# samedii/perceptor

Measured on AMD Instinct MI355X. Metric: denoising steps/sec (UNet+CLIP-grad) at 512x512 batch 8, higher is better.
Workload: dtype bf16

## Files before the change

### perceptor_amd/csrc/build.py

```python
from __future__ import annotations

import os
import subprocess
import sys
from concurrent.futures import ThreadPoolExecutor

HERE = os.path.dirname(os.path.abspath(__file__))
LIB = os.path.join(HERE, "libperceptor_hip.so")
SOURCES = ["igemm.hip", "conv3x3.hip", "conv_wd.hip", "gemm_wd.hip", "norm.hip", "attn.hip", "attn_flash.hip", "elementwise.hip", "clip.hip", "f32gemm.hip", "sampling.hip", "backward.hip", "resnet.hip"]
FLAGS = ["-O3", "--offload-arch=gfx950", "-std=c++17", "-fPIC"]
FILE_FLAGS = {"conv_wd.hip": ["-fno-slp-vectorize"]}


def _stale(out: str, deps) -> bool:
    if not os.path.exists(out):
        return True
    t = os.path.getmtime(out)
    return any(os.path.getmtime(d) > t for d in deps)


def build(force: bool = False, verbose: bool = False, variant: str = "", extra_flags=()) -> str:
    hipcc = os.environ.get("HIPCC", "/opt/rocm/bin/hipcc")
    lib = LIB if not variant else LIB.replace(".so", f"_{variant}.so")
    bdir = "build" if not variant else f"build_{variant}"
    hdrs = [os.path.join(HERE, "common.h"), os.path.join(HERE, "..", "..", "include", "perceptor_hip.h")]
    srcs = [s for s in SOURCES if os.path.exists(os.path.join(HERE, s))]
    objs = []

    def compile_one(src):
        obj = os.path.join(HERE, bdir, src.replace(".hip", ".o"))
        os.makedirs(os.path.dirname(obj), exist_ok=True)
        if force or _stale(obj, [os.path.join(HERE, src)] + hdrs):
            cmd = [hipcc, *FLAGS, *FILE_FLAGS.get(src, []), *extra_flags, "-c", os.path.join(HERE, src), "-o", obj]
            if verbose:
                print(" ".join(cmd), flush=True)
            subprocess.run(cmd, check=True)
        return obj

    with ThreadPoolExecutor(max_workers=min(7, len(srcs))) as ex:
        objs = list(ex.map(compile_one, srcs))
    if force or _stale(lib, objs):
        cmd = [hipcc, "--offload-arch=gfx950", "-shared", "-fPIC", "-o", lib, *objs]
        if verbose:
            print(" ".join(cmd), flush=True)
# ... 10 lines not shown
```

### perceptor_amd/csrc/conv3x3.hip

```cpp
#include "common.h"
#include "epilogue.h"
#include "../../include/perceptor_hip.h"

namespace {

constexpr int PW = 34;

__device__ __forceinline__ int swz(int row, int chunk) { return row * 128 + ((chunk ^ ((row >> 1) & 7)) << 4); }

template <typename T, int WM, int WN, int PRO, bool EARLY, int NJ = 4, int NWB = 2>
__global__ __launch_bounds__(WM * WN * 64, 2) void conv3x3_halo_kernel(const pmi_igemm_args a) {
  constexpr int XB = 2;
  constexpr int TH = WM * XB;
  constexpr int NT = WM * WN * 64;
  constexpr int RPI = NT / 8;
  constexpr int BN = WN * NJ * 32;
  constexpr int PP = (TH + 2) * PW;
  constexpr int NPI = (PP + RPI - 1) / RPI;
  constexpr int NWI = BN / RPI;
  constexpr int PATCH_BYTES = NPI * RPI * 128;
  constexpr int WBYTES = BN * 128;
  __shared__ __attribute__((aligned(16))) char smem[PATCH_BYTES + NWB * WBYTES];
  char* const wbuf = smem + PATCH_BYTES;

// ... 322 lines not shown
    const int tiles = nimg * (a.H / 8) * (a.W / 32) * ((a.N + 31) / 32);
    hipLaunchKernelGGL((conv3x3_halo_kernel<T, 4, 1, PRO, false, 1>), dim3(tiles), dim3(256), 0, s, a);
  } else {
    const int tiles = nimg * (a.H / 8) * (a.W / 32) * ((a.N + 127) / 128);
    hipLaunchKernelGGL((conv3x3_halo_kernel<T, 4, 1, PRO, false>), dim3(tiles), dim3(256), 0, s, a);
  }
  PMI_CHECK_LAUNCH();
  return PMI_OK;
}

template <typename T>
int launch_t(const pmi_igemm_args& a, hipStream_t s, int cfg) {
  if (!a.pro_a) return launch_p<T, 0>(a, s, cfg);
  switch (a.pro_act) {
    case PMI_ACT_NONE: return launch_p<T, 1 + PMI_ACT_NONE>(a, s, cfg);
    case PMI_ACT_RELU: return launch_p<T, 1 + PMI_ACT_RELU>(a, s, cfg);
    case PMI_ACT_SILU: return launch_p<T, 1 + PMI_ACT_SILU>(a, s, cfg);
    default: return PMI_ERR_ARG;
  }
}

}

static int g_prefer0 = 1;
static int g_force_cfg = -1;
static int g_wd = 1;
static int g_wd128 = 1;
static int g_wd_mf16 = 1;
void pmi_conv3x3_allow_wd(int v) { g_wd = v; }
void pmi_conv3x3_wd_mf16(int v) { g_wd_mf16 = v; }
void pmi_conv3x3_wd128(int v) { g_wd128 = v; }
static int g_wd_smallc = 1;
void pmi_conv3x3_wd_smallc(int v) { g_wd_smallc = v; }
void pmi_conv3x3_force_config(int cfg) { g_force_cfg = cfg; }
void pmi_conv3x3_prefer_256(int v) { g_prefer0 = v; }

extern "C" int pmi_conv3x3_halo_config(const pmi_igemm_args* a) {
  if (a->taps != 9 || a->stride != 1 || a->batch > 1) return -1;
  const int Cin = a->C0 + a->C1;
  if (a->Bf && g_wd && g_wd_mf16 && g_wd_smallc && a->C1 == 0 && !a->A1 && a->C0 <= 32 && (a->C0 % 8) == 0 && !a->up && (a->W % 32) == 0 && (a->H % 8) == 0 && !a->pro_a &&
      ((!a->split_out && !a->split_in) || (a->split_out == 32 && a->split_in == 1 && (a->N % 128) == 0 && a->dtype != PMI_DT_BF16)) &&
      !a->out_f32 && !(a->R && a->res_f32) && (a->N % 32) == 0 && a->N >= 64 && (g_force_cfg < 0 || g_force_cfg == 8) &&
      (long)(a->M / (a->H * a->W)) * (a->H / 8) * (a->W / 32) * ((a->N + 127) / 128) >= (g_force_cfg == 8 ? 1 : 256))
    return 8;
  if ((Cin % 64) || (a->C0 % 64) || (a->W % 32) || (a->H % 8)) return -1;
  const bool plain_k = a->split_in == 1 && !a->split_out && !a->pro_a && a->out_f32 && a->N <= 32;
  if ((a->split_out || a->split_in) && !plain_k) {
    if (!a->Bf || !g_wd || !g_wd_mf16 || a->split_out != 32 || a->out_f32 || (a->N % 128) || a->dtype == PMI_DT_BF16) return -1;
    if (a->split_in == 2 && !a->pro_a) return -1;
    if (a->pro_a && (a->pro_act != PMI_ACT_SILU || !a->split_in)) return -1;
    const int cin_l = a->split_in == 1 ? Cin / 2 : Cin;
    const int t8s = a->M / (a->H * a->W) * (a->H / 8) * (a->W / 32);
    const bool ok6 = (a->N % 256) == 0 && (!a->pro_a || cin_l <= 2048), ok7 = !a->pro_a || cin_l <= 1024;
    if (g_force_cfg == 6 || g_force_cfg == 7) return (g_force_cfg == 6 ? ok6 : ok7) ? g_force_cfg : -1;
    if (g_force_cfg >= 0) return -1;
    if (ok6 && t8s * (a->N / 256) >= 192) return 6;
    if (g_wd128 && ok7 && t8s * (a->N / 128) >= 128) return 7;
    return -1;
  }
  if (a->N <= 32 && (a->N % 4) == 0 && !a->stats && !a->res_up && a->M / (a->H * a->W) * (a->H / 8) * (a->W / 32) >= 256) return 3;
  if (a->out_f32 || (a->R && a->res_f32)) return -1;
  if (a->N % 128) {
    const int t8 = a->M / (a->H * a->W) * (a->H / 8) * (a->W / 32);
    const bool ok7t = a->Bf && g_wd && g_wd_mf16 && (a->N % 32) == 0 && (a->N % 128) >= 64 && a->N > 128 && (!a->pro_a || a->C0 + a->C1 <= 1024);
    if (g_force_cfg == 7) return ok7t ? 7 : -1;
    return (g_force_cfg < 0 && g_wd128 && ok7t && t8 * ((a->N + 127) / 128) >= 256) ? 7 : -1;
  }
  if (a->Bf && g_wd && (!a->pro_a || a->C0 + a->C1 <= 2048)) {
    const int t8 = a->M / (a->H * a->W) * (a->H / 8) * (a->W / 32);
    const bool ok4 = (a->N % 256) == 0;
    if (g_force_cfg == 4 && ok4) return 4;
    if (g_force_cfg == 6 && ok4) return 6;
    if (g_force_cfg < 0 && ok4 && t8 * (a->N / 256) >= 192) return g_wd_mf16 ? 6 : 4;
    const bool ok7 = g_wd_mf16 && (!a->pro_a || a->C0 + a->C1 <= 1024);
    if (g_force_cfg == 7 && ok7) return 7;
    if (g_force_cfg < 0 && g_wd128 && ok7 && !ok4 && t8 * (a->N / 128) >= (a->N > 512 ? 128 : 256)) return 7;
    if (g_force_cfg < 0 && g_wd128 && ok7 && ok4 && t8 * (a->N / 128) >= 128) return 7;
  }
  const bool ok0 = (a->N % 256) == 0 || a->N >= 256, ok1 = (a->H % 16) == 0;
  if (g_force_cfg == 0 && ok0) return 0;
  if (g_force_cfg == 1 && ok1) return 1;
  if (g_force_cfg == 2) return 2;
  const int nimg = a->M / (a->H * a->W);
  const int px_tiles8 = nimg * (a->H / 8) * (a->W / 32);
  if (g_prefer0 && (a->N % 256) == 0 && px_tiles8 * (a->N / 256) >= 256) return 0;
  if (px_tiles8 * (a->N / 128) >= 128) return 2;
  if ((a->N % 256) == 0) return px_tiles8 * (a->N / 256) >= 192 ? 0 : -1;
  if (ok1 && (px_tiles8 / 2) * (a->N / 128) >= 192) return 1;
  return -1;
}

int pmi_conv3x3_halo_launch(const pmi_igemm_args* a, int cfg, void* stream) {
  hipStream_t s = (hipStream_t)stream;
  return a->dtype == PMI_DT_BF16 ? launch_t<BF16>(*a, s, cfg) : launch_t<F16>(*a, s, cfg);
}
```

### perceptor_amd/csrc/igemm.hip

```cpp
#include <cstdio>
#include <cstdlib>
#include "common.h"
#include "epilogue.h"
#include "../../include/perceptor_hip.h"

namespace {

constexpr int BM = 128, BN = 128, BK = 64;
constexpr int TILE_BYTES = 128 * 128;
constexpr int STAGE_BYTES = 2 * TILE_BYTES;

__device__ __forceinline__ int lds_off(int row, int chunk) { return row * 128 + ((chunk ^ ((row >> 1) & 7)) << 4); }

template <typename T, bool CONV, bool KFAST, bool PHASED = false>
__global__ __launch_bounds__(256, 2) void igemm_kernel(const pmi_igemm_args a) {
  static_assert(!PHASED || CONV, "the phased geometry is a convolution");
  __shared__ __attribute__((aligned(16))) char smem[2 * STAGE_BYTES];

  const int tid = threadIdx.x, lane = tid & 63, wid = tid >> 6;
  const int wr = wid >> 1, wc = wid & 1;
#ifdef PMI_STAMPS
#define GSTAMP(k) do { if (tid == 0 && a.reserved == 77 && a.splitk <= 1) ((long long*)a.ws)[(int64_t)blockIdx.x * 8 + (k)] = (long long)wall_clock64(); } while (0)
#else
#define GSTAMP(k) do {} while (0)
// ... 477 lines not shown
template <typename T>
int launch(const pmi_igemm_args& a, hipStream_t s) {
  const bool phased = a.up == 2;
  const int tiles = (((phased ? a.M / 4 : a.M) + BM - 1) / BM) * ((a.N + BN - 1) / BN);
  const dim3 grid(tiles, phased ? 4 : 1, a.batch > 1 ? a.batch : (a.splitk > 1 ? a.splitk : 1)), block(256);
  const bool conv = a.taps != 1 || a.up || a.stride == 2;
  const int Cin = a.C0 + a.C1;
  const bool kfast = (Cin % BK == 0) && (a.C0 % BK == 0);
  if (phased) {
    if (kfast) hipLaunchKernelGGL((igemm_kernel<T, true, true, true>), grid, block, 0, s, a);
    else hipLaunchKernelGGL((igemm_kernel<T, true, false, true>), grid, block, 0, s, a);
  } else if (conv) {
    if (kfast) hipLaunchKernelGGL((igemm_kernel<T, true, true>), grid, block, 0, s, a);
    else hipLaunchKernelGGL((igemm_kernel<T, true, false>), grid, block, 0, s, a);
  } else {
    if (kfast) hipLaunchKernelGGL((igemm_kernel<T, false, true>), grid, block, 0, s, a);
    else hipLaunchKernelGGL((igemm_kernel<T, false, false>), grid, block, 0, s, a);
  }
  PMI_CHECK_LAUNCH();
  if (a.splitk > 1) {
    const int64_t work = (int64_t)a.M * (a.N / 4);
    const int blocks = (int)((work + 255) / 256 > 4096 ? 4096 : (work + 255) / 256);
    hipLaunchKernelGGL(splitk_reduce_kernel<T>, dim3(blocks), dim3(256), 0, s, a);
    PMI_CHECK_LAUNCH();
  }
  return PMI_OK;
}

}

extern "C" int pmi_conv3x3_halo_config(const pmi_igemm_args* a);
int pmi_conv3x3_halo_launch(const pmi_igemm_args* a, int cfg, void* stream);
int pmi_conv3x3_wd_launch(const pmi_igemm_args* a, int cfg, void* stream);
extern "C" int pmi_gemm_wd_eligible(const pmi_igemm_args* a);
int pmi_gemm_wd_tile_rows(const pmi_igemm_args* a, int splitk);
int pmi_gemm_wd_launch(const pmi_igemm_args* a, void* stream);
void pmi_conv3x3_allow_wd(int v);
void pmi_conv3x3_wd_mf16(int v);
void pmi_conv3x3_wd128(int v);
void pmi_conv3x3_force_config(int cfg);
void pmi_conv3x3_prefer_256(int v);
static int g_allow_halo = 1;
static int g_wd_max_split = 8;
int pmi_conv3x3_wd_splitk(const pmi_igemm_args* a, int cfg);
extern "C" int pmi_igemm_splitk(const pmi_igemm_args* a) {
  if (a->batch > 1 || (a->N & 3) || a->up == 2) return 1;
  if (g_allow_halo) {
    const int halo = pmi_conv3x3_halo_config(a);
    if (halo >= 0) return pmi_conv3x3_wd_splitk(a, halo);
  }
  if (a->act == PMI_ACT_GEGLU) return 1;
  if (a->A1 && a->taps == 1 && pmi_gemm_wd_eligible(a)) return 1;
  if (pmi_gemm_wd_eligible(a)) {
    const int nch = (a->K + 127) / 128;
    int best = 1;
    long best_cost = -1;
    for (int s = 1; s <= g_wd_max_split && nch / s >= 4; s *= 2) {
      const int rows = pmi_gemm_wd_tile_rows(a, s);
      const long wgs = (long)((a->M + rows - 1) / rows) * (a->N < 256 ? 1 : (a->N + 255) / 256) * s;
      const long cost = ((wgs + 255) / 256) * rows * (nch / s + 6) + (s > 1 ? 8L * 144 : 0);
      if (best_cost < 0 || cost < best_cost) { best_cost = cost; best = s; }
    }
    return best;
  }
  const int tiles = ((a->M + BM - 1) / BM) * ((a->N + BN - 1) / BN);
  const int nk = (a->K + BK - 1) / BK;
  if (tiles >= 384 || nk < 16) return 1;
  int s = 512 / tiles;
  if (s > nk / 8) s = nk / 8;
  if (s > 16) s = 16;
  return s < 2 ? 1 : s;
}

int pmi_igemm_halo_allowed(void) { return g_allow_halo; }

extern "C" int pmi_igemm_stats_rows(const pmi_igemm_args* a) {
  if (a->batch > 1 || a->splitk > 1 || a->up == 2) return 0;
  const int halo = g_allow_halo ? pmi_conv3x3_halo_config(a) : -1;
  if (a->split_out) return halo >= 6 ? (a->H / 8) * (a->W / 32) : 0;
  if (halo == 3) return 0;
  if (halo >= 0) return (a->H / (halo == 1 ? 16 : 8)) * (a->W / 32);
  if (a->hw > 0 && (a->hw % BM) == 0 && (a->M % a->hw) == 0) return a->hw / BM;
  return 0;
}

void pmi_attn_flash_qt(int v);
void pmi_attn_flash_kv_chunks(int v);
void pmi_conv3x3_wd_splitk_enable(int v);
void pmi_gemm_wd_few_wgs(int v);
void pmi_conv3x3_wd_smallc(int v);

extern "C" int pmi_set_option(int key, int value) {
  if (key == 0) { const int old = g_allow_halo; g_allow_halo = value; return old; }
  if (key == 1) { pmi_conv3x3_force_config(value); return 0; }
  if (key == 2) { pmi_conv3x3_prefer_256(value); return 0; }
  if (key == 6) { pmi_conv3x3_allow_wd(value); return 0; }
  if (key == 7) { pmi_conv3x3_wd_mf16(value); return 0; }
  if (key == 8) { pmi_conv3x3_wd128(value); return 0; }
  if (key == 9) { pmi_attn_flash_qt(value); return 0; }
  if (key == 10) { pmi_conv3x3_wd_splitk_enable(value); return 0; }
  if (key == 11) { g_wd_max_split = value; return 0; }
  if (key == 12) { pmi_gemm_wd_few_wgs(value); return 0; }
  if (key == 13) { pmi_conv3x3_wd_smallc(value); return 0; }
  if (key == 14) { pmi_attn_flash_kv_chunks(value); return 0; }
  return PMI_ERR_ARG;
}

static int bad_arg(int line) {
  if (getenv("PMI_DEBUG")) fprintf(stderr, "pmi_igemm: argument check at igemm.hip:%d failed\n", line);
  return PMI_ERR_ARG;
}

extern "C" int pmi_igemm(const pmi_igemm_args* a, pmi_stream_t stream) {
  if (!a || !a->A0 || !a->B || !a->D) return bad_arg(__LINE__);
  if (a->M <= 0 || a->N <= 0 || a->K <= 0) return bad_arg(__LINE__);
  if ((a->K & 7) || (a->C0 & 7) || (a->C1 & 7)) return bad_arg(__LINE__);
  if ((a->N & 3) && (a->bias || a->nbias || a->R || a->ldd < ((a->N + 3) & ~3))) return bad_arg(__LINE__);
  if ((a->lda0 & 7) || (a->ldb & 7) || (a->ldd & 3)) return bad_arg(__LINE__);
  if (a->C1 > 0 && (!a->A1 || (a->lda1 & 7))) return bad_arg(__LINE__);
  if (a->taps != 1 && a->taps != 9 && a->taps != 16) return bad_arg(__LINE__);
  if (a->taps == 16 && (a->stride != 2 || a->up || a->res_up || a->Hin != 2 * a->H || a->Win != 2 * a->W)) return bad_arg(__LINE__);
  if (a->stride != 1 && a->stride != 2) return bad_arg(__LINE__);
  if (a->up == 2 && (a->taps != 9 || a->stride != 2 || a->res_up || a->A1 || a->C1 || a->R || a->nbias || a->stats || a->splitk > 1 || a->batch > 1 ||
                     a->split_out || a->split_in || a->pro_a || a->D2 || a->aux || a->dtype == PMI_DT_F16X2 || (a->M & 3))) return bad_arg(__LINE__);
  if (a->K != a->taps * (a->C0 + a->C1)) return bad_arg(__LINE__);
  if (a->R && (a->ldr & 3)) return bad_arg(__LINE__);
  if (a->split_out && ((a->split_out & 7) || a->split_out > 32 || a->out_f32 || (a->N % a->split_out) || a->batch > 1)) return bad_arg(__LINE__);
  if ((unsigned)a->split_in > 2u) return bad_arg(__LINE__);
  if (a->split_in == 2 && !a->split_out) return bad_arg(__LINE__);
  if (a->nbias && a->hw <= 0) return bad_arg(__LINE__);
  const bool conv = a->taps != 1 || a->up || a->stride == 2;
  if (a->res_up && ((a->H & 1) || (a->W & 1))) return bad_arg(__LINE__);
  if ((conv || a->res_up) && (a->H <= 0 || a->W <= 0 || a->Hin <= 0 || a->Win <= 0 || a->M % (a->H * a->W))) return bad_arg(__LINE__);
  if (a->up && (a->H != 2 * a->Hin || a->W != 2 * a->Win)) return bad_arg(__LINE__);
  if (a->batch > 1 && a->batch_inner <= 0) return bad_arg(__LINE__);
  const int halo = g_allow_halo ? pmi_conv3x3_halo_config(a) : -1;
  if (a->pro_a && (!a->pro_b || halo < 0)) return PMI_ERR_ARG;
  if ((a->split_in == 2 || ((a->split_in || a->split_out) && a->pro_a) || (a->split_out && a->R && a->res_f32)) && halo < 6) return bad_arg(__LINE__);
  if (a->stats && a->stats_p != pmi_igemm_stats_rows(a)) return PMI_ERR_ARG;
  if (a->splitk > 1 && (!a->ws || a->batch > 1 || (halo >= 0 && a->splitk != pmi_conv3x3_wd_splitk(a, halo)) || (a->N & 3) || a->stats)) return PMI_ERR_ARG;
  if (a->act == PMI_ACT_GEGLU && !pmi_gemm_wd_eligible(a)) return bad_arg(__LINE__);
  if ((a->D2 || a->aux) && !pmi_gemm_wd_eligible(a)) return bad_arg(__LINE__);
  if (pmi_gemm_wd_eligible(a) && !((a->nbias || a->res_up) && a->splitk <= 1)) {
    const int rc = pmi_gemm_wd_launch(a, stream);
    if (rc != PMI_OK || a->splitk <= 1 || a->reserved3 == 1) return rc;
    hipStream_t s = (hipStream_t)stream;
    const int64_t work = (int64_t)a->M * (a->N / 4);
    const int blocks = (int)((work + 255) / 256 > 4096 ? 4096 : (work + 255) / 256);
    if (a->dtype == PMI_DT_BF16) hipLaunchKernelGGL(splitk_reduce_kernel<BF16>, dim3(blocks), dim3(256), 0, s, *a);
    else hipLaunchKernelGGL(splitk_reduce_kernel<F16>, dim3(blocks), dim3(256), 0, s, *a);
    PMI_CHECK_LAUNCH();
    return PMI_OK;
  }
  if (halo >= 4) {
    const int rc = pmi_conv3x3_wd_launch(a, halo, stream);
    if (rc != PMI_OK || a->splitk <= 1) return rc;
    hipStream_t s = (hipStream_t)stream;
    const int64_t work = (int64_t)a->M * (a->N / 4);
    const int blocks = (int)((work + 255) / 256 > 4096 ? 4096 : (work + 255) / 256);
    if (a->dtype == PMI_DT_BF16) hipLaunchKernelGGL(splitk_reduce_kernel<BF16>, dim3(blocks), dim3(256), 0, s, *a);
    else hipLaunchKernelGGL(splitk_reduce_kernel<F16>, dim3(blocks), dim3(256), 0, s, *a);
    PMI_CHECK_LAUNCH();
    return PMI_OK;
  }
  if (halo >= 0) return pmi_conv3x3_halo_launch(a, halo, stream);
  hipStream_t s = (hipStream_t)stream;
  return a->dtype == PMI_DT_BF16 ? launch<BF16>(*a, s) : launch<F16>(*a, s);
}

extern "C" int pmi_abi_version(void) { return 1; }
```

### perceptor_amd/engine/adm.py

```python
from __future__ import annotations

from dataclasses import dataclass
from typing import Dict, List, Optional, Tuple

import torch

from .. import _hip
from .._hip import ACT_NONE, ACT_SILU, call, ptr
from . import ops
from .ops import PackedLinear


@dataclass(frozen=True)
class AdmConfig:
    image_size: int
    model_channels: int
    num_res_blocks: int
    channel_mult: Tuple[float, ...]
    attention_ds: Tuple[int, ...]
    num_heads: int = 1
    num_head_channels: int = -1
    num_heads_upsample: int = -1
    use_scale_shift_norm: bool = False
    resblock_updown: bool = False
# ... 113 lines not shown
                S[p + ".qkv.weight"] = (3 * l.c, l.c, 1); S[p + ".qkv.bias"] = (3 * l.c,)
                S[p + ".proj_out.weight"] = (l.c, l.c, 1); S[p + ".proj_out.bias"] = (l.c,)
            elif isinstance(l, _Resample) and cfg.conv_resample:
                n = l.p + (".conv" if l.up else ".op")
                S[n + ".weight"] = (l.c, l.c, 3, 3); S[n + ".bias"] = (l.c,)
    S["out.0.weight"] = (ch_last,); S["out.0.bias"] = (ch_last,)
    S["out.2.weight"] = (cfg.out_channels, int(cfg.channel_mult[0] * mc), 3, 3); S["out.2.bias"] = (cfg.out_channels,)
    return S


class AdmEngine:
    def __init__(self, cfg: AdmConfig, state_dict: Dict[str, torch.Tensor], device, dtype="bf16"):
        self.cfg, self.device = cfg, torch.device(device)
        self.dt = _hip.dtype_code(dtype)
        _hip.lib()
        sd, dev, dt = state_dict, self.device, self.dt
        self.inp, self.mid, self.out, self.ch_last = build_plan(cfg)
        f32 = lambda k: sd[k].detach().float().to(dev).contiguous()
        lin = lambda k, **kw: PackedLinear(sd[k + ".weight"], sd.get(k + ".bias"), dt, dev, **kw)
        self.w: Dict[str, object] = {}
        self.precise = dt == _hip.DT_F16X2
        if self.precise:
            self.te0, self.te2 = (f32("time_embed.0.weight"), f32("time_embed.0.bias")), (f32("time_embed.2.weight"), f32("time_embed.2.bias"))
        else:
            self.te0, self.te2 = lin("time_embed.0"), lin("time_embed.2")
        emb_w, emb_b, off = [], [], 0
        for layers in self.inp + [self.mid] + self.out:
            for l in layers:
                if isinstance(l, tuple):
                    self.w[l[1]] = lin(l[1], cin_pad=8)
                elif isinstance(l, _Res):
                    p = l.p
                    self.w[p + ".gn1"] = (f32(p + ".in_layers.0.weight"), f32(p + ".in_layers.0.bias"))
                    self.w[p + ".conv1"] = lin(p + ".in_layers.2", sources=l.srcs)
                    self.w[p + ".gn2"] = (f32(p + ".out_layers.0.weight"), f32(p + ".out_layers.0.bias"))
                    self.w[p + ".conv2"] = lin(p + ".out_layers.3")
                    if l.cin != l.cout:
                        self.w[p + ".skip"] = lin(p + ".skip_connection", sources=l.srcs)
                    l.emb_off = off
                    emb_w.append(sd[p + ".emb_layers.1.weight"].float()); emb_b.append(sd[p + ".emb_layers.1.bias"].float())
                    off += emb_w[-1].shape[0]
                elif isinstance(l, _Attn):
                    p = l.p
                    self.w[p + ".gn"] = (f32(p + ".norm.weight"), f32(p + ".norm.bias"))
                    self.w[p + ".qkv"] = lin(p + ".qkv")
                    self.w[p + ".proj"] = lin(p + ".proj_out")
                elif isinstance(l, _Resample) and cfg.conv_resample:
                    self.w[l.p] = lin(l.p + (".conv" if l.up else ".op"))
        if self.precise:
            self.emb_all = (torch.cat(emb_w, 0).to(dev).contiguous(), torch.cat(emb_b, 0).to(dev).contiguous())
        else:
            self.emb_all = PackedLinear(torch.cat(emb_w, 0), torch.cat(emb_b, 0), dt, dev)
        self.gn_out = (f32("out.0.weight"), f32("out.0.bias"))
        self.conv_out = lin("out.2")

    def _res(self, l: _Res, x, x1, emb):
        cfg, dt, w = self.cfg, self.dt, self.w
        g1, b1 = w[l.p + ".gn1"]
        ecols = 2 * l.cout if cfg.use_scale_shift_norm else l.cout
        e = emb[:, l.emb_off:l.emb_off + ecols]
        nb = None if cfg.use_scale_shift_norm else e
        skip, skip1 = x, x1
        if l.down:
            if x1 is None:
                h, skip = ops.group_norm_pool_skip(x, g1, b1, 32, dt, act=ACT_SILU)
            else:
                h = ops.group_norm(x, g1, b1, 32, dt, x1=x1, act=ACT_SILU, pool=True)
                skip = ops.avgpool2(x, dt)
            h = ops.igemm(h, w[l.p + ".conv1"], nbias=nb, want_stats=True)
        else:
            ca, cb = ops.group_norm_coeffs(x, g1, b1, 32, dt, x1=x1)
            h = ops.igemm(x, w[l.p + ".conv1"], a1=x1, up=l.up, nbias=nb, prologue=(ca, cb, ACT_SILU), want_stats=True)
        g2, b2 = w[l.p + ".gn2"]
        if cfg.use_scale_shift_norm:
            ca, cb = ops.group_norm_coeffs(h, g2, b2, 32, dt, film=e, film_ld=emb.stride(0))
        else:
            ca, cb = ops.group_norm_coeffs(h, g2, b2, 32, dt)
        if l.cin != l.cout:
            skip = ops.igemm(skip, w[l.p + ".skip"], a1=skip1)
        elif skip1 is not None:
            raise NotImplementedError("identity skip over a concatenated input does not occur in the shipped configs")
# ... 246 lines not shown
```

### perceptor_amd/engine/ops.py

```python
from __future__ import annotations

import math
import os
import ctypes as C
from typing import Optional

import torch

from .. import _hip
from .._hip import ACT_GEGLU, ACT_NONE, DT_F16X2, IgemmArgs, call, ptr


HALO_ENABLED = True
SPLITK_ENABLED = True
WD_ENABLED = True
GEMM_WD_ENABLED = True
GEMM_WD_CONV = os.environ.get("PMI_GEMM_WD_CONV", "1") != "0"
FLASH_ENABLED = True


def set_halo(enabled: bool) -> None:
    global HALO_ENABLED
    HALO_ENABLED = bool(enabled)
    _hip.lib().pmi_set_option(0, int(enabled))


KERNEL_EVENTS = None
GEMM_TRACE = None
DEBUG_WS = None


def _empty(shape, dtype, device):
    return torch.empty(shape, dtype=dtype, device=device)


def split_group(c: int) -> int:
    if c % 32 == 0:
        return 32
    if c > 32 or c % 8:
        raise ValueError(f"precise tensors need a channel count that is a multiple of 32 (or of 8 below 32), got {c}")
    return c


def logical_c(x: torch.Tensor, dt: int) -> int:
    return x.shape[-1] // 2 if dt == DT_F16X2 else x.shape[-1]


class PackedLinear:

    def __init__(self, weight: torch.Tensor, bias: Optional[torch.Tensor], dt: int, device, cin_pad: Optional[int] = None, sources=None,
                 concat_sources: bool = True):
        w = weight.detach().float()
        if w.ndim == 3:
            w = w[..., 0]
        if w.ndim == 2:
            w = w[:, :, None, None]
        cout, cin, kh, kw = w.shape
        self.cout, self.cin, self.taps = cout, cin, kh * kw
        self.cin_p = cin_pad if cin_pad is not None else (cin + 7) // 8 * 8
        self.n_p = (cout + 3) // 4 * 4
        packed = torch.zeros(self.n_p, kh * kw, self.cin_p, dtype=torch.float32)
        packed[:cout, :, :cin] = w.permute(0, 2, 3, 1).reshape(cout, kh * kw, cin)
        self.split = dt == DT_F16X2
        self.cin_l = self.cin_p
        self.self_concat = False
        self.concat_inputs = False
        if self.split:
            def dup(wt, lo_zero=False):
                parts, o = [], 0
                for cs in (sources or [self.cin_l]):
                    g = split_group(cs)
                    blk = wt[:, :, o:o + cs].reshape(self.n_p, kh * kw, cs // g, 1, g).expand(-1, -1, -1, 2, -1).clone()
                    if lo_zero:
                        blk[:, :, :, 1, :] = 0
                    parts.append(blk.reshape(self.n_p, kh * kw, 2 * cs))
                    o += cs
                assert o == self.cin_l
                return torch.cat(parts, dim=2)
            w_hi = packed.to(torch.float16).float()
            w_lo = packed - w_hi
            self._w1, self._sources = w_hi, list(sources or [self.cin_l])
            packed = dup(w_hi)
            self.cin_p = 2 * self.cin_l
            if float(w_lo.norm()) > 2.0 ** -22 * float(w_hi.norm()):
                concat_ok = sources is None or (concat_sources and all(cs % 32 == 0 for cs in sources))
                if not concat_ok:
                    import warnings
                    warnings.warn("precise mode: fp32 weights of a two-source (concat) convolution are rounded to f16")
                else:
                    packed = torch.cat([packed, dup(w_lo, lo_zero=True)], dim=2)
                    self.self_concat = True
                    self.concat_inputs = sources is not None
                    self.cin_p = 2 * self.cin_p
        self.w = packed.reshape(self.n_p, -1).to(device=device, dtype=_hip.TORCH_DTYPE[dt]).contiguous()
        self.b = None
        if bias is not None:
            b = torch.zeros(self.n_p, dtype=torch.float32)
            b[:cout] = bias.detach().float()
            self.b = b.to(device)
        self.dt = dt
        self._frag = {}

    @property
    def K(self):
        return self.taps * self.cin_p

    def frag_gemm(self) -> torch.Tensor:
        if "gemm" not in self._frag:
            assert self.taps in (1, 9) and self.n_p % 32 == 0 and self.K % 32 == 0
            kp = (self.K + 127) // 128 * 128
            w = self.w
            if kp != self.K:
                w = torch.zeros((self.n_p, kp), dtype=self.w.dtype, device=self.w.device)
                w[:, :self.K] = self.w
            w = w.view(self.n_p // 32, 2, 16, kp // 128, 4, 4, 8)
            self._frag["gemm"] = w.permute(0, 3, 4, 1, 5, 2, 6).contiguous()
        return self._frag["gemm"]

    def frag16(self, ck: int, dup_g: int = 0) -> torch.Tensor:
        key = ("mf16", ck, dup_g)
        if key not in self._frag:
            assert self.taps == 9 and self.n_p % 32 == 0 and self.cin_p % ck == 0
            src = self.w
            if dup_g and dup_g != 32:
                assert self.split and not self.self_concat and all(cs % dup_g == 0 for cs in self._sources)
                parts, o = [], 0
                for cs in self._sources:
                    blk = self._w1[:, :, o:o + cs].reshape(self.n_p, 9, cs // dup_g, 1, dup_g).expand(-1, -1, -1, 2, -1)
                    parts.append(blk.reshape(self.n_p, 9, 2 * cs))
                    o += cs
                src = torch.cat(parts, dim=2).reshape(self.n_p, -1).to(device=self.w.device, dtype=self.w.dtype).contiguous()
            w = src.view(self.n_p // 32, 2, 16, 3, 3, self.cin_p // ck, ck // 32, 4, 8)
            self._frag[key] = w.permute(0, 5, 4, 6, 3, 1, 7, 2, 8).contiguous()
        return self._frag[key]
# ... 182 lines not shown
        m = n * h * w
        a.H, a.W, a.Hin, a.Win = h, w, hin, win
        a.hw = h * w
        oshape = (n, h, w, lin.n_p)
    else:
        assert lin.taps == 1 and not up and stride == 1
        m = a0.shape[0]
        a.hw = hw or 1
        oshape = (m, lin.n_p // 2 if act == ACT_GEGLU else lin.n_p)
    if lin.split:
        a.split_in = 1
    if (lin.split and not out_f32) or split_out:
        a.split_out = split_group(lin.n_p)
        oshape = oshape[:-1] + (2 * lin.n_p,)
    if out is None:
        out = _empty(oshape, torch.float32 if out_f32 else _hip.TORCH_DTYPE[dt], a0.device)
    a.A0, a.A1, a.B = ptr(a0), ptr(a1), ptr(lin.w)
    a.bias, a.nbias, a.R, a.D = ptr(lin.b), ptr(nbias), ptr(residual), ptr(out)
    a.M, a.N, a.K = m, lin.n_p, lin.K
    a.C0, a.C1 = c0, c1
    a.lda0, a.lda1 = a0.stride(-2), (a1.stride(-2) if a1 is not None else 0)
    a.ldb, a.ldd = lin.K, out.stride(-2)
    a.ldr = residual.stride(-2) if residual is not None else 0
    a.taps, a.stride, a.up, a.res_up, a.act = lin.taps, stride, int(up), int(res_up), act
    a.out_f32 = int(out.dtype == torch.float32)
    a.res_f32 = int(residual is not None and residual.dtype == torch.float32)
    a.alpha = alpha
    a.ldnb = nbias.stride(0) if nbias is not None else 0
    a.batch, a.batch_inner = 1, 1
    a.dtype = dt
    if conv and lin.taps == 9 and stride == 1 and HALO_ENABLED and WD_ENABLED and lin.n_p % 32 == 0 and ((lin.n_p >= 128 and lin.cin_p % 64 == 0) or (lin.cin_p <= 32 and a1 is None)):
        a.Bf = 1
        a.pro_a = 1 if (prologue is not None and not lin.split) else None
        cfg = _hip.lib().pmi_conv3x3_halo_config(C.byref(a))
        a.pro_a = None
        a.Bf = ptr(lin.frag16(64)) if cfg == 6 else ptr(lin.frag16(32)) if cfg == 7 else ptr(lin.frag(64)) if cfg == 4 else ptr(lin.frag_c8()) if cfg == 8 else None
    if pre_out is not None or act_grad_of is not None:
        a.D2, a.aux, a.aux_act = ptr(pre_out), ptr(act_grad_of), act_grad
    wd_ok = GEMM_WD_ENABLED and lin.taps == 1 and (not lin.split or out_f32) and not up and stride == 1 and lin.n_p % 32 == 0 and lin.K % 32 == 0 \
        and nbias is None and prologue is None
    if wd_ok and want_stats:
        wd_ok = SPLITK_ENABLED and _hip.lib().pmi_igemm_splitk(C.byref(a)) > 1
    if wd_ok:
        a.Bf = 1
        a.Bf = ptr(lin.frag_gemm()) if _hip.lib().pmi_gemm_wd_eligible(C.byref(a)) else None
        if a.Bf:
            want_stats = False
    if prologue is not None:
        ca, cb, pact = prologue
        if HALO_ENABLED and not lin.split and _hip.lib().pmi_conv3x3_halo_config(C.byref(a)) >= 0:
            a.pro_a, a.pro_b, a.pro_act = ptr(ca), ptr(cb), pact
        else:
            if lin.split and a1 is not None and (c0 // 2) % 32 + (c1 // 2) % 32:
                raise ValueError(f"precise two-source prologue: sources of {c0 // 2} + {c1 // 2} channels are not both multiples of 32")
            n_, h_, w_, _ = a0.shape
            y = _empty((n_, h_, w_, c0 + c1), a0.dtype, a0.device)
            lc0, lc = (c0 // 2, (c0 + c1) // 2) if lin.split else (c0, c0 + c1)
            call("pmi_gn_apply", ptr(a0), ptr(a1), lc0, ptr(ca), ptr(cb), None, ptr(y), n_, h_, w_, lc, pact, 0, dt)
            a.A0, a.A1, a.C0, a.C1, a.lda0, a.lda1 = ptr(y), None, c0 + c1, 0, c0 + c1, 0
            a0 = y
    if lin.self_concat:
        assert a.A1 is None
        a.A1, a.C1, a.lda1 = a.A0, a.C0, a.lda0
    conv_gemm = False
    if conv and lin.taps == 9 and stride == 1 and not up and GEMM_WD_ENABLED and GEMM_WD_CONV and not lin.split and not a.Bf \
            and not a.pro_a and lin.n_p % 32 == 0 and c0 % 128 == 0 and c1 % 128 == 0:
        a.Bf = 1
        a.Bf = ptr(lin.frag_gemm()) if _hip.lib().pmi_gemm_wd_eligible(C.byref(a)) else None
        conv_gemm = bool(a.Bf)
# ... 629 lines not shown
```

Before: 25.12.

## Add sub-pixel phase-decomposed 2x upsample conv3x3 kernel with pre-summed 2x2 weights

Adds a new kernel for a nearest-2x upsample followed by a 3x3 conv. It splits the output into four sub-pixel phases, and each phase becomes a 2x2 conv over the low-resolution input using pre-summed effective weights, packed at load time. This cuts the MAC count from 9 taps to 4 per output and avoids reading the upsampled input. It costs a new selection path (config 9), a four-fold weight pack held in memory, and a large new kernel whose correctness and perf tuning are unproven.

Measured after the change: 25.97 (median of 6 runs). 3.4% higher.

```diff
diff --git a/perceptor_amd/csrc/build.py b/perceptor_amd/csrc/build.py
--- a/perceptor_amd/csrc/build.py
+++ b/perceptor_amd/csrc/build.py
@@ -7,9 +7,9 @@
 
 HERE = os.path.dirname(os.path.abspath(__file__))
 LIB = os.path.join(HERE, "libperceptor_hip.so")
-SOURCES = ["igemm.hip", "conv3x3.hip", "conv_wd.hip", "gemm_wd.hip", "norm.hip", "attn.hip", "attn_flash.hip", "elementwise.hip", "clip.hip", "f32gemm.hip", "sampling.hip", "backward.hip", "resnet.hip"]
+SOURCES = ["igemm.hip", "conv3x3.hip", "conv_wd.hip", "conv_up_wd.hip", "gemm_wd.hip", "norm.hip", "attn.hip", "attn_flash.hip", "elementwise.hip", "clip.hip", "f32gemm.hip", "sampling.hip", "backward.hip", "resnet.hip"]
 FLAGS = ["-O3", "--offload-arch=gfx950", "-std=c++17", "-fPIC"]
-FILE_FLAGS = {"conv_wd.hip": ["-fno-slp-vectorize"]}
+FILE_FLAGS = {"conv_wd.hip": ["-fno-slp-vectorize"], "conv_up_wd.hip": ["-fno-slp-vectorize"]}
 
 
 def _stale(out: str, deps) -> bool:
diff --git a/perceptor_amd/csrc/conv3x3.hip b/perceptor_amd/csrc/conv3x3.hip
--- a/perceptor_amd/csrc/conv3x3.hip
+++ b/perceptor_amd/csrc/conv3x3.hip
@@ -378,6 +378,8 @@
 void pmi_conv3x3_wd128(int v) { g_wd128 = v; }
 static int g_wd_smallc = 1;
 void pmi_conv3x3_wd_smallc(int v) { g_wd_smallc = v; }
+static int g_up_phase = 1;
+void pmi_conv3x3_up_phase(int v) { g_up_phase = v; }
 void pmi_conv3x3_force_config(int cfg) { g_force_cfg = cfg; }
 void pmi_conv3x3_prefer_256(int v) { g_prefer0 = v; }
 
@@ -412,6 +414,10 @@
     if (g_force_cfg == 7) return ok7t ? 7 : -1;
     return (g_force_cfg < 0 && g_wd128 && ok7t && t8 * ((a->N + 127) / 128) >= 256) ? 7 : -1;
   }
+  if (a->Bf && g_wd && g_wd_mf16 && g_up_phase && a->up == 1 && !a->A1 && a->C1 == 0 && !a->R && !a->split_in && !a->split_out && a->act == PMI_ACT_NONE &&
+      a->reserved3 != 2 && (a->N % 256) == 0 && (a->Win % 32) == 0 && (a->Hin % 8) == 0 && (!a->pro_a || a->C0 <= 2048) &&
+      (g_force_cfg == 9 || (g_force_cfg < 0 && (long)(a->M / (a->H * a->W)) * (a->Hin / 8) * (a->Win / 32) * 4 * (a->N / 256) >= 192)))
+    return 9;
   if (a->Bf && g_wd && (!a->pro_a || a->C0 + a->C1 <= 2048)) {
     const int t8 = a->M / (a->H * a->W) * (a->H / 8) * (a->W / 32);
     const bool ok4 = (a->N % 256) == 0;
diff --git a/perceptor_amd/csrc/conv_up_wd.hip b/perceptor_amd/csrc/conv_up_wd.hip
--- /dev/null
+++ b/perceptor_amd/csrc/conv_up_wd.hip
@@ -0,0 +1,335 @@
+#include "common.h"
+#include "../../include/perceptor_hip.h"
+
+#ifndef UP_FINE
+#define UP_FINE 2
+#endif
+#ifndef UP_FROW
+#define UP_FROW 1
+#endif
+
+namespace {
+
+constexpr int PW = 33, PR = 9;
+
+template <typename T, int PRO>
+__global__ __launch_bounds__(512, 2) void conv3x3_up_wd_kernel(const pmi_igemm_args a) {
+  constexpr int NW = 8, NT = 512, CK = 64, KS = 2;
+  constexpr int PP = PR * PW;
+  constexpr int CPR = CK / 8;
+  constexpr int NG = 2 * KS * 2;
+  constexpr int WGC = 2 * KS;
+  constexpr int NWF = 4;
+  constexpr int GB = NWF * 1024;
+  constexpr int NPI = (PP * CPR + NT - 1) / NT;
+  constexpr int ROW = CK * 2 + 32;
+  constexpr int PATCH_BYTES = (NPI * NT / CPR) * ROW;
+  constexpr int BN = 256, NPX = 256;
+  constexpr int SROW = BN * 2 + 16;
+  constexpr int EPI_BYTES = NPX * SROW + NW * BN * 8 + BN * 4;
+  constexpr int MAXCIN = 2048;
+  constexpr int CTAB = MAXCIN + 8;
+  constexpr int COEF_BYTES = PRO ? 2 * CTAB * 4 : 0;
+  constexpr int PPIX_BYTES = NPI * NT * 4;
+  static_assert(NPI <= NG - 1, "the next patch must be complete before the barrier in the chunk's last group");
+  constexpr int BSM_OFF = (2 * PATCH_BYTES + COEF_BYTES + PPIX_BYTES) > (EPI_BYTES - BN * 4) ? (2 * PATCH_BYTES + COEF_BYTES + PPIX_BYTES) : (EPI_BYTES - BN * 4);
+  static_assert(BSM_OFF + BN * 4 <= 160 * 1024, "LDS budget");
+  static_assert(15 * ROW + 48 + 16 + (ROW + 64 + 16 * ROW) + 8 * PW * ROW <= PATCH_BYTES, "fragment reads stay inside a patch buffer");
+  __shared__ __attribute__((aligned(16))) char smem[BSM_OFF + BN * 4];
+  float* const bsm = (float*)(smem + BSM_OFF);
+  float* const coef = (float*)(smem + 2 * PATCH_BYTES);
+  int* const ppix_s = (int*)(smem + 2 * PATCH_BYTES + COEF_BYTES);
+
+  const int tid = threadIdx.x, lane = tid & 63;
+  if (PRO && tid < 16) coef[(tid >> 3) * CTAB + MAXCIN + (tid & 7)] = 0.f;
+  const int wid = __builtin_amdgcn_readfirstlane(tid >> 6);
+  const int wn = wid;
+
+  const int tiles_x = a.Win / 32, tiles_y = a.Hin / 8, tiles_n = a.N / BN;
+  const int nimg = a.M / (a.H * a.W);
+  int logical = xcd_remap(blockIdx.x, nimg * tiles_y * tiles_x * tiles_n * 4);
+  const int phase = logical & 3; logical >>= 2;
+  const int tn = logical % tiles_n; logical /= tiles_n;
+  const int tx = logical % tiles_x; logical /= tiles_x;
+  const int ty = logical % tiles_y;
+  const int img = logical / tiles_y;
+  const int pa = phase >> 1, pb_ = phase & 1;
+  const int y0 = ty * 8, x0 = tx * 32, n0 = tn * BN;
+
+#ifdef PMI_STAMPS
+#define STAMP(k) do { if (tid == 0 && a.ws) ((long long*)a.ws)[(int64_t)blockIdx.x * 8 + (k)] = (long long)wall_clock64(); } while (0)
+#else
+#define STAMP(k) do {} while (0)
+#endif
+  STAMP(0);
+  const int Cin = a.C0;
+  const int nchunks = Cin / CK;
+  const int sc = tid % CPR;
+  const int64_t img_px = (int64_t)a.Hin * a.Win;
+  const u16* const A0i = (const u16*)a.A0 + (int64_t)img * img_px * a.lda0;
+  const __amdgpu_buffer_rsrc_t rs_a = make_rsrc(A0i, ((img_px - 1) * a.lda0 + a.C0) * 2);
+  const uint32_t ld2 = (uint32_t)a.lda0 * 2u;
+  const int64_t wslab = (int64_t)nchunks * WGC * GB;
+  const __amdgpu_buffer_rsrc_t rsrc_w = make_rsrc((const char*)a.Bf + ((int64_t)(tn * NW + wn) * 4 + phase) * wslab, wslab);
+  const uint32_t wvo = (uint32_t)lane * 16u;
+
+#pragma unroll
+  for (int i = 0; i < NPI; ++i) {
+    const int pp = tid / CPR + (NT / CPR) * i;
+    const int py = pp / PW, px = pp - py * PW;
+    const int sy = y0 - 1 + pa + py, sx = x0 - 1 + pb_ + px;
+    const bool inside = pp < PP && (unsigned)sy < (unsigned)a.Hin && (unsigned)sx < (unsigned)a.Win;
+    ppix_s[i * NT + tid] = inside ? sy * a.Win + sx : -1;
+  }
+
+  auto load_piece = [&](int chunk, int pix, bool live) -> uint4 {
+    const uint32_t vo = (pix >= 0 && live) ? (uint32_t)pix * ld2 + (uint32_t)sc * 16u : PMI_BUF_OOB;
+    return buf_load16(rs_a, vo, (uint32_t)(chunk * CK) * 2u);
+  };
+  constexpr bool PSILU = PRO == 1 + PMI_ACT_SILU;
+  constexpr float NLOG2E = -1.4426950408889634f;
+  auto read_coef = [&](int chunk, int pix, float* ga, float* gb) {
+    const float* ca = coef + (pix >= 0 ? chunk * CK + sc * 8 : MAXCIN);
+    *(float4*)ga = *(const float4*)ca; *(float4*)(ga + 4) = *(const float4*)(ca + 4);
+    *(float4*)gb = *(const float4*)(ca + CTAB); *(float4*)(gb + 4) = *(const float4*)(ca + CTAB + 4);
+  };
+  auto cvt_piece = [&](uint4 pc, int pix, const float* ga, const float* gb, bool mask) -> uint4 {
+    if (!PRO) return pc;
+    float f[8];
+    unpack8<T>(pc, f);
+#pragma unroll
+    for (int e = 0; e < 8; ++e) {
+      if constexpr (PSILU) {
+        const float u = __builtin_fmaf(f[e], ga[e], gb[e]);
+        f[e] = u * __builtin_amdgcn_rcpf(__builtin_fmaf(__builtin_amdgcn_exp2f(u), NLOG2E, NLOG2E));
+      } else {
+        f[e] = act_apply(f[e] * ga[e] + gb[e], PRO - 1);
+      }
+    }
+    const uint32_t keep = (!mask || pix >= 0) ? 0xffffffffu : 0u;
+    uint4 v = pack8<T>(f);
+    v.x &= keep; v.y &= keep; v.z &= keep; v.w &= keep;
+    return v;
+  };
+  auto write_piece = [&](char* pbuf, int i, const uint4& o) {
+    *(uint4*)(pbuf + (tid / CPR) * ROW + sc * 16 + i * (NT / CPR) * ROW) = o;
+  };
+
+  f32x4 acc4[8][2][2];
+#pragma unroll
+  for (int i = 0; i < 8; ++i)
+#pragma unroll
+    for (int r = 0; r < 16; ++r) acc4[i][(r >> 3) & 1][(r >> 2) & 1][r & 3] = 0.f;
+
+  for (int c = tid; c < BN; c += NT) {
+    const int n = n0 + c;
+    float b = 0.f;
+    if (a.bias) b = a.bias[n];
+    if (a.nbias) b += a.nbias[(int64_t)img * (a.ldnb ? a.ldnb : a.N) + n];
+    bsm[c] = b;
+  }
+
+  uint4 wq[2][NWF];
+  auto load_wg = [&](int slot, int group) {
+    const uint32_t vo = wvo + (uint32_t)group * (uint32_t)GB;
+#pragma unroll
+    for (int f = 0; f < NWF; ++f) wq[slot][f] = buf_load16(rsrc_w, vo + f * 1024u, 0);
+  };
+
+  load_wg(0, 0);
+  {
+    uint4 p0[NPI];
+    float ga[8], gb[8];
+#pragma unroll
+    for (int i = 0; i < NPI; ++i) p0[i] = load_piece(0, ppix_s[i * NT + tid], true);
+    if (PRO) {
+      for (int c = tid; c < Cin; c += NT) {
+        coef[c] = a.pro_a[(int64_t)img * Cin + c] * (PSILU ? NLOG2E : 1.f);
+        coef[CTAB + c] = a.pro_b[(int64_t)img * Cin + c] * (PSILU ? NLOG2E : 1.f);
+      }
+      __syncthreads();
+      read_coef(0, 0, ga, gb);
+    }
+#pragma unroll
+    for (int i = 0; i < NPI; ++i) write_piece(smem, i, cvt_piece(p0[i], ppix_s[i * NT + tid], ga, gb, true));
+  }
+  __syncthreads();
+  STAMP(1);
+
+  const int frag0 = (lane & 15) * ROW + (lane >> 4) * 16;
+  auto goff = [&](int g) -> int { const int q = g >> 1, s = g & 1; return (q / KS) * ROW + (q % KS) * 64 + s * 16 * ROW; };
+  static_assert((3 * NG) % 6 == 0, "fragment window must repeat per chunk");
+  uint4 xf[6];
+#pragma unroll
+  for (int r = 0; r < 6; ++r) xf[r] = *(const uint4*)(smem + frag0 + r * PW * ROW);
+  int pixc = ppix_s[0 * NT + tid];
+  uint4 pr = load_piece(nchunks > 1 ? 1 : 0, pixc, nchunks > 1);
+  int pixn = ppix_s[1 * NT + tid];
+  for (int chunk = 0; chunk < nchunks; ++chunk) {
+    const char* const pb = smem + (chunk & 1) * PATCH_BYTES;
+    char* const pn = smem + ((chunk + 1) & 1) * PATCH_BYTES;
+    const bool more = chunk + 1 < nchunks;
+    const int cn = more ? chunk + 1 : chunk;
+    const bool more2 = chunk + 2 < nchunks;
+    const int cn2 = more2 ? chunk + 2 : chunk;
+    const int gbase = chunk * WGC;
+#pragma unroll
+    for (int g = 0; g < NG; ++g) {
+      if (g & 1) load_wg(((g >> 1) + 1) & 1, gbase + (g >> 1) + 1);
+      const bool store_slot = g < NPI;
+      const int lp = (g + 1 == NG) ? 0 : g + 1;
+      const bool load_slot = (g + 1 == NG) || lp < NPI;
+      float ga[8], gb[8];
+      if (PRO && store_slot) read_coef(cn, pixc, ga, gb);
+      uint4 prn = pr;
+      int pixl = pixc;
+      if (load_slot) { prn = load_piece(lp == 0 ? cn2 : cn, pixn, lp == 0 ? more2 : more); pixl = pixn; }
+      __builtin_amdgcn_sched_barrier(0);
+      uint4 po;
+      if (store_slot) {
+        if (PRO) po = cvt_piece(pr, pixc, ga, gb, false);
+        else write_piece(pn, g, pr);
+      }
+      const char* const cb0 = pb + frag0 + goff(g);
+      const char* const nb = (g + 1 < NG ? pb : pn) + frag0 + goff((g + 1) % NG);
+      auto rows = [&](int i0, int i1) {
+#pragma unroll
+        for (int i = i0; i < i1; ++i) {
+#pragma unroll
+          for (int dy = 0; dy < 2; ++dy)
+#pragma unroll
+            for (int cb = 0; cb < 2; ++cb)
+              acc4[i][g & 1][cb] = T::mfma16(wq[(g >> 1) & 1][dy * 2 + cb], xf[(i + dy + 3 * g) % 6], acc4[i][g & 1][cb]);
+          if (i < 3) xf[(i + 3 * g) % 6] = *(const uint4*)(cb0 + (i + 6) * PW * ROW);
+          else if (i < 7) xf[(i + 3 * g) % 6] = *(const uint4*)(nb + (i - 3) * PW * ROW);
+          else {
+            xf[(7 + 3 * g) % 6] = *(const uint4*)(nb + 4 * PW * ROW);
+            xf[(8 + 3 * g) % 6] = *(const uint4*)(nb + 5 * PW * ROW);
+          }
+        }
+#pragma unroll
+        for (int i = i0; i < i1; ++i) {
+          if (UP_FINE && PRO && store_slot && i >= UP_FROW) {
+#pragma unroll
+            for (int m = 0; m < 4; ++m) {
+              __builtin_amdgcn_sched_group_barrier(0x008, 1, 0);
+              __builtin_amdgcn_sched_group_barrier(0x002, UP_FINE, 0);
+            }
+            __builtin_amdgcn_sched_group_barrier(0x100, 1, 0);
+          } else {
+            __builtin_amdgcn_sched_group_barrier(0x008, 4, 0);
+            __builtin_amdgcn_sched_group_barrier(0x100, 1, 0);
+          }
+        }
+      };
+      if (g == NG - 1) {
+        rows(0, 3);
+        __builtin_amdgcn_sched_barrier(0);
+        __syncthreads();
+        __builtin_amdgcn_sched_barrier(0);
+        rows(3, 8);
+      } else {
+        rows(0, 8);
+      }
+      __builtin_amdgcn_sched_group_barrier(0x100, 1, 0);
+      if (PRO && store_slot) write_piece(pn, g, po);
+      int pixn2 = pixn;
+      if (load_slot) pixn2 = ppix_s[((lp + 1) % NPI) * NT + tid];
+      pr = prn; pixc = pixl; pixn = pixn2;
+      __builtin_amdgcn_sched_barrier(0);
+    }
+  }
+  STAMP(2);
+
+  char* const stg = smem;
+  float* const stat = (float*)(smem + NPX * SROW);
+  constexpr int LPR = BN / 8;
+  constexpr int PPI = 64 / LPR;
+  constexpr int PXW = NPX / NW;
+  constexpr int NWI = PXW / PPI;
+  const int q = lane % LPR, psub = lane / LPR;
+  const int cl0 = q * 8;
+  const __amdgpu_buffer_rsrc_t rs_d = make_rsrc((u16*)a.D + (int64_t)img * a.H * a.W * a.ldd, ((int64_t)(a.H * a.W - 1) * a.ldd + a.N) * 2);
+  const uint32_t dvo = (uint32_t)(psub * 2 * a.ldd + n0 + cl0) * 2u;
+  {
+    float4 bb[2];
+#pragma unroll
+    for (int cb = 0; cb < 2; ++cb) bb[cb] = *(const float4*)(bsm + wn * 32 + cb * 16 + 4 * (lane >> 4));
+#pragma unroll
+    for (int i = 0; i < 8; ++i)
+#pragma unroll
+      for (int sx = 0; sx < 2; ++sx)
+#pragma unroll
+        for (int cb = 0; cb < 2; ++cb) {
+          const int cl = wn * 32 + cb * 16 + 4 * (lane >> 4);
+          const float4 b = bb[cb];
+          const f32x4 c = acc4[i][sx][cb];
+          *(uint2*)(stg + (i * 32 + sx * 16 + (lane & 15)) * SROW + cl * 2) =
+              pack4<T>(c[0] * a.alpha + b.x, c[1] * a.alpha + b.y, c[2] * a.alpha + b.z, c[3] * a.alpha + b.w);
+        }
+  }
+  __syncthreads();
+  STAMP(6);
+  float cs[16];
+#pragma unroll
+  for (int e = 0; e < 16; ++e) cs[e] = 0.f;
+  const uint32_t orow = (uint32_t)((2 * (y0 + wid) + pa) * a.W + 2 * x0 + pb_);
+#pragma unroll
+  for (int t = 0; t < NWI; ++t) {
+    const int p = wid * PXW + t * PPI + psub;
+    const uint4 v = *(const uint4*)(stg + p * SROW + cl0 * 2);
+    if (a.stats) {
+      float f[8];
+      unpack8<T>(v, f);
+#pragma unroll
+      for (int e = 0; e < 8; ++e) { cs[e] += f[e]; cs[8 + e] += f[e] * f[e]; }
+    }
+    buf_store16_nt(v, rs_d, dvo, (orow + (uint32_t)(2 * t * PPI)) * (uint32_t)a.ldd * 2u);
+  }
+  STAMP(7);
+  if (a.stats) {
+#pragma unroll
+    for (int e = 0; e < 16; ++e) cs[e] += __shfl_xor(cs[e], 32);
+    if (lane < LPR) {
+      float* const slot = stat + (wid * BN + cl0) * 2;
+#pragma unroll
+      for (int e = 0; e < 8; ++e) { slot[2 * e] = cs[e]; slot[2 * e + 1] = cs[8 + e]; }
+    }
+    __syncthreads();
+    float* o = a.stats + (((int64_t)img * a.stats_p + (ty * tiles_x + tx) * 4 + phase) * a.N + n0) * 2;
+    for (int c = tid; c < 2 * BN; c += NT) {
+      float v = 0.f;
+#pragma unroll
+      for (int w = 0; w < NW; ++w) v += stat[w * 2 * BN + c];
+      o[c] = v;
+    }
+  }
+#ifdef PMI_STAMPS
+  __syncthreads();
+  STAMP(3);
+  STAMP(4);
+#endif
+}
+
+template <typename T>
+int launch_t(const pmi_igemm_args& a, hipStream_t s) {
+  const dim3 grid((a.M / (a.H * a.W)) * (a.Hin / 8) * (a.Win / 32) * 4 * (a.N / 256));
+  if (!a.pro_a) hipLaunchKernelGGL((conv3x3_up_wd_kernel<T, 0>), grid, dim3(512), 0, s, a);
+  else if (a.pro_act == PMI_ACT_SILU) hipLaunchKernelGGL((conv3x3_up_wd_kernel<T, 1 + PMI_ACT_SILU>), grid, dim3(512), 0, s, a);
+  else if (a.pro_act == PMI_ACT_RELU) hipLaunchKernelGGL((conv3x3_up_wd_kernel<T, 1 + PMI_ACT_RELU>), grid, dim3(512), 0, s, a);
+  else if (a.pro_act == PMI_ACT_NONE) hipLaunchKernelGGL((conv3x3_up_wd_kernel<T, 1 + PMI_ACT_NONE>), grid, dim3(512), 0, s, a);
+  else return PMI_ERR_ARG;
+  PMI_CHECK_LAUNCH();
+  return PMI_OK;
+}
+
+}
+
+int pmi_conv3x3_up_wd_launch(const pmi_igemm_args* a, void* stream) {
+  if (!a->Bf || a->up != 1 || a->taps != 9 || a->stride != 1 || a->A1 || a->C1 || a->R || a->split_in || a->split_out || a->out_f32 || a->splitk > 1 ||
+      a->act != PMI_ACT_NONE || (a->N % 256) || (a->C0 % 64) || (a->Win % 32) || (a->Hin % 8) || a->H != 2 * a->Hin || a->W != 2 * a->Win ||
+      (a->pro_a && a->C0 > 2048))
+    return PMI_ERR_ARG;
+  hipStream_t s = (hipStream_t)stream;
+  return a->dtype == PMI_DT_BF16 ? launch_t<BF16>(*a, s) : launch_t<F16>(*a, s);
+}
diff --git a/perceptor_amd/csrc/igemm.hip b/perceptor_amd/csrc/igemm.hip
--- a/perceptor_amd/csrc/igemm.hip
+++ b/perceptor_amd/csrc/igemm.hip
@@ -533,6 +533,7 @@
 extern "C" int pmi_conv3x3_halo_config(const pmi_igemm_args* a);
 int pmi_conv3x3_halo_launch(const pmi_igemm_args* a, int cfg, void* stream);
 int pmi_conv3x3_wd_launch(const pmi_igemm_args* a, int cfg, void* stream);
+int pmi_conv3x3_up_wd_launch(const pmi_igemm_args* a, void* stream);
 extern "C" int pmi_gemm_wd_eligible(const pmi_igemm_args* a);
 int pmi_gemm_wd_tile_rows(const pmi_igemm_args* a, int splitk);
 int pmi_gemm_wd_launch(const pmi_igemm_args* a, void* stream);
@@ -590,6 +591,7 @@
 void pmi_conv3x3_wd_splitk_enable(int v);
 void pmi_gemm_wd_few_wgs(int v);
 void pmi_conv3x3_wd_smallc(int v);
+void pmi_conv3x3_up_phase(int v);
 
 extern "C" int pmi_set_option(int key, int value) {
   if (key == 0) { const int old = g_allow_halo; g_allow_halo = value; return old; }
@@ -604,6 +606,7 @@
   if (key == 12) { pmi_gemm_wd_few_wgs(value); return 0; }
   if (key == 13) { pmi_conv3x3_wd_smallc(value); return 0; }
   if (key == 14) { pmi_attn_flash_kv_chunks(value); return 0; }
+  if (key == 15) { pmi_conv3x3_up_phase(value); return 0; }
   return PMI_ERR_ARG;
 }
 
@@ -653,6 +656,7 @@
     PMI_CHECK_LAUNCH();
     return PMI_OK;
   }
+  if (halo == 9) return pmi_conv3x3_up_wd_launch(a, stream);
   if (halo >= 4) {
     const int rc = pmi_conv3x3_wd_launch(a, halo, stream);
     if (rc != PMI_OK || a->splitk <= 1) return rc;
diff --git a/perceptor_amd/engine/adm.py b/perceptor_amd/engine/adm.py
--- a/perceptor_amd/engine/adm.py
+++ b/perceptor_amd/engine/adm.py
@@ -169,7 +169,7 @@
                 elif isinstance(l, _Res):
                     p = l.p
                     self.w[p + ".gn1"] = (f32(p + ".in_layers.0.weight"), f32(p + ".in_layers.0.bias"))
-                    self.w[p + ".conv1"] = lin(p + ".in_layers.2", sources=l.srcs)
+                    self.w[p + ".conv1"] = lin(p + ".in_layers.2", sources=l.srcs, up_phase=l.up)
                     self.w[p + ".gn2"] = (f32(p + ".out_layers.0.weight"), f32(p + ".out_layers.0.bias"))
                     self.w[p + ".conv2"] = lin(p + ".out_layers.3")
                     if l.cin != l.cout:
@@ -183,7 +183,7 @@
                     self.w[p + ".qkv"] = lin(p + ".qkv")
                     self.w[p + ".proj"] = lin(p + ".proj_out")
                 elif isinstance(l, _Resample) and cfg.conv_resample:
-                    self.w[l.p] = lin(l.p + (".conv" if l.up else ".op"))
+                    self.w[l.p] = lin(l.p + (".conv" if l.up else ".op"), up_phase=l.up)
         if self.precise:
             self.emb_all = (torch.cat(emb_w, 0).to(dev).contiguous(), torch.cat(emb_b, 0).to(dev).contiguous())
         else:
diff --git a/perceptor_amd/engine/ops.py b/perceptor_amd/engine/ops.py
--- a/perceptor_amd/engine/ops.py
+++ b/perceptor_amd/engine/ops.py
@@ -49,7 +49,7 @@
 class PackedLinear:
 
     def __init__(self, weight: torch.Tensor, bias: Optional[torch.Tensor], dt: int, device, cin_pad: Optional[int] = None, sources=None,
-                 concat_sources: bool = True):
+                 concat_sources: bool = True, up_phase: bool = False):
         w = weight.detach().float()
         if w.ndim == 3:
             w = w[..., 0]
@@ -100,6 +100,25 @@
             self.b = b.to(device)
         self.dt = dt
         self._frag = {}
+        if up_phase and not self.split and kh == 3 and kw == 3 and self.n_p % 256 == 0 and self.cin_p % 64 == 0:
+            self._frag[("up", 64)] = self._pack_up(packed.view(self.n_p, 3, 3, self.cin_p), 64, device, dt)
+
+    @staticmethod
+    def _pack_up(w: torch.Tensor, ck: int, device, dt: int) -> torch.Tensor:
+        n, _, _, cin = w.shape
+        rows = torch.stack([torch.stack([w[:, 0], w[:, 1] + w[:, 2]], 1), torch.stack([w[:, 0] + w[:, 1], w[:, 2]], 1)], 1)
+        eff = torch.stack([torch.stack([rows[:, :, :, 0], rows[:, :, :, 1] + rows[:, :, :, 2]], 3),
+                           torch.stack([rows[:, :, :, 0] + rows[:, :, :, 1], rows[:, :, :, 2]], 3)], 2)
+        eff = eff.to(device=device, dtype=_hip.TORCH_DTYPE[dt])
+        e = eff.view(n // 32, 2, 16, 2, 2, 2, 2, cin // ck, ck // 32, 4, 8)
+        return e.permute(0, 3, 4, 7, 6, 8, 5, 1, 9, 2, 10).contiguous()
+
+    def frag16_up(self, ck: int) -> Optional[torch.Tensor]:
+        return self._frag.get(("up", ck))
+
+    def up_weights(self) -> torch.Tensor:
+        f = self._frag[("up", 64)]
+        return f.permute(0, 7, 9, 1, 2, 6, 4, 3, 5, 8, 10).reshape(self.n_p, 2, 2, 2, 2, self.cin_p)
 
     @property
     def K(self):
@@ -348,9 +367,11 @@
     if conv and lin.taps == 9 and stride == 1 and HALO_ENABLED and WD_ENABLED and lin.n_p % 32 == 0 and ((lin.n_p >= 128 and lin.cin_p % 64 == 0) or (lin.cin_p <= 32 and a1 is None)):
         a.Bf = 1
         a.pro_a = 1 if (prologue is not None and not lin.split) else None
+        if up and lin.frag16_up(64) is None:
+            a.reserved3 = 2
         cfg = _hip.lib().pmi_conv3x3_halo_config(C.byref(a))
         a.pro_a = None
-        a.Bf = ptr(lin.frag16(64)) if cfg == 6 else ptr(lin.frag16(32)) if cfg == 7 else ptr(lin.frag(64)) if cfg == 4 else ptr(lin.frag_c8()) if cfg == 8 else None
+        a.Bf = ptr(lin.frag16_up(64)) if cfg == 9 else ptr(lin.frag16(64)) if cfg == 6 else ptr(lin.frag16(32)) if cfg == 7 else ptr(lin.frag(64)) if cfg == 4 else ptr(lin.frag_c8()) if cfg == 8 else None
     if pre_out is not None or act_grad_of is not None:
         a.D2, a.aux, a.aux_act = ptr(pre_out), ptr(act_grad_of), act_grad
     wd_ok = GEMM_WD_ENABLED and lin.taps == 1 and (not lin.split or out_f32) and not up and stride == 1 and lin.n_p % 32 == 0 and lin.K % 32 == 0 \
```
